# balazs-bamer/cdpr-simulation

Measured on AMD Instinct MI355X. Metric: CDPR sim-steps/sec (whole node), 65 536 parallel 8-cable robots, 1 ms dt, higher is better.
Workload: dtype f32

## Files before the change

cdpr-simulation_amd/csrc/cdpr_engine.hip:

```cpp
#include "cdpr_engine_internal.hpp"

namespace {
thread_local std::string g_create_error;
}

namespace cdpr_host {

int derivative_weights(uint32_t n, uint32_t degree, double* w) {
  if (n < 2 || n > CDPR_MAX_D_BUFFER || degree < 1 || degree > CDPR_MAX_D_DEGREE || degree >= n) return CDPR_ERR_INVALID;
  const int m = (int)degree + 1;
  long double a[5][10];
  for (int i = 0; i < m; ++i)
    for (int j = 0; j < 2 * m; ++j) a[i][j] = 0.0L;
  std::vector<long double> x(n);
  for (uint32_t j = 0; j < n; ++j) x[j] = (long double)j - (long double)(n - 1) / 2.0L;
  for (int i = 0; i < m; ++i) {
    for (int k = 0; k < m; ++k) {
      long double s = 0;
      for (uint32_t j = 0; j < n; ++j) s += powl(x[j], i + k);
      a[i][k] = s;
    }
    a[i][m + i] = 1.0L;
  }
  for (int col = 0; col < m; ++col) {
// ... 497 lines not shown
  HIP_TRY(h, hipMemcpyAsync(c.d_mask, mask.data(), B, hipMemcpyHostToDevice, h->stream));
  HIP_TRY(h, wait_stream(h));
  c.pending = true;
  c.masked = true;
  return CDPR_OK;
}

static int set_command(cdpr_engine* h, int kind, const float* axes, size_t count, bool from_device) {
  if (!h) return CDPR_ERR_INVALID;
  const int rc = stage_command(h, kind, axes, count, from_device);
  if (rc == CDPR_OK) {
    CmdChannel& c = h->cmd[kind];
    c.pending = true;
    c.masked = false;
    c.ext[1] = nullptr;
  }
  return rc;
}

static int bind_command(cdpr_engine* h, int kind, const float* d_axes, size_t count) {
  if (!h) return CDPR_ERR_INVALID;
  if (!d_axes) {
    h->err = "null command buffer";
    return CDPR_ERR_INVALID;
  }
  if (count != (size_t)h->n * h->batch) return CDPR_IGNORED;
  if (h->plan.per_robot) {
    h->err = "cdpr_bind_*_command_device: not available on a per_robot_commands handle (commands are latched robot by robot)";
    return CDPR_ERR_UNSUPPORTED;
  }
  h->cmd[kind].ext[1] = d_axes;
  h->cmd[kind].pending = true;
  return CDPR_OK;
}

int cdpr_set_velocity_command(cdpr_handle_t h, const float* axes, size_t count) { return set_command(h, CDPR_COMMAND_VELOCITY, axes, count, false); }
int cdpr_set_position_command(cdpr_handle_t h, const float* axes, size_t count) { return set_command(h, CDPR_COMMAND_POSITION, axes, count, false); }
int cdpr_set_force_command(cdpr_handle_t h, const float* axes, size_t count) { return set_command(h, CDPR_COMMAND_FORCE, axes, count, false); }

int cdpr_set_velocity_command_device(cdpr_handle_t h, const float* d_axes, size_t count) { return set_command(h, CDPR_COMMAND_VELOCITY, d_axes, count, true); }
int cdpr_set_position_command_device(cdpr_handle_t h, const float* d_axes, size_t count) { return set_command(h, CDPR_COMMAND_POSITION, d_axes, count, true); }
int cdpr_set_force_command_device(cdpr_handle_t h, const float* d_axes, size_t count) { return set_command(h, CDPR_COMMAND_FORCE, d_axes, count, true); }

int cdpr_set_velocity_command_masked(cdpr_handle_t h, const float* axes, size_t count, const uint8_t* robot_mask) {
  return stage_masked(h, CDPR_COMMAND_VELOCITY, axes, count, robot_mask);
}
int cdpr_set_position_command_masked(cdpr_handle_t h, const float* axes, size_t count, const uint8_t* robot_mask) {
  return stage_masked(h, CDPR_COMMAND_POSITION, axes, count, robot_mask);
}
int cdpr_set_force_command_masked(cdpr_handle_t h, const float* axes, size_t count, const uint8_t* robot_mask) {
  return stage_masked(h, CDPR_COMMAND_FORCE, axes, count, robot_mask);
}

int cdpr_bind_velocity_command_device(cdpr_handle_t h, const float* d_axes, size_t count) { return bind_command(h, CDPR_COMMAND_VELOCITY, d_axes, count); }
int cdpr_bind_position_command_device(cdpr_handle_t h, const float* d_axes, size_t count) { return bind_command(h, CDPR_COMMAND_POSITION, d_axes, count); }
int cdpr_bind_force_command_device(cdpr_handle_t h, const float* d_axes, size_t count) { return bind_command(h, CDPR_COMMAND_FORCE, d_axes, count); }

int cdpr_update(cdpr_handle_t h, int nsteps) { return run_steps(h, nsteps, 1); }

int cdpr_update_fused(cdpr_handle_t h, int nsteps, int steps_per_launch) { return run_steps(h, nsteps, steps_per_launch); }

int cdpr_observable_image_bytes(cdpr_handle_t h, size_t* bytes) {
  if (!h || !bytes) return CDPR_ERR_INVALID;
  *bytes = image_bytes(h);
  return CDPR_OK;
}

int cdpr_update_record(cdpr_handle_t h, int nsteps, int steps_per_launch, void* d_record, size_t record_bytes) {
  if (!h) return CDPR_ERR_INVALID;
  if (h->cfg.publish_period != 0.0) {
    h->err = "cdpr_update_record needs publish_period == 0 (every step published)";
    return CDPR_ERR_UNSUPPORTED;
  }
  const size_t image = image_bytes(h);
  if (!d_record || nsteps < 0 || record_bytes < image * (size_t)nsteps) {
    h->err = "cdpr_update_record: record buffer missing or smaller than nsteps observable images";
    return CDPR_ERR_INVALID;
  }
  return run_steps(h, nsteps, steps_per_launch, d_record);
}

int cdpr_update_scheduled(cdpr_handle_t h, int nsteps, int refresh_steps, const float* d_commands, const uint32_t* d_ready, void* d_record,
                          size_t record_bytes) {
  if (!h) return CDPR_ERR_INVALID;
  return scheduled_update(h, CDPR_COMMAND_VELOCITY, nsteps, refresh_steps, d_commands, d_ready, nullptr, d_record, record_bytes);
}

int cdpr_update_scheduled_kind(cdpr_handle_t h, uint32_t kind, int nsteps, int refresh_steps, const float* d_commands, const uint32_t* d_ready,
                               const uint8_t* d_robot_masks, void* d_record, size_t record_bytes) {
  if (!h) return CDPR_ERR_INVALID;
  return scheduled_update(h, kind, nsteps, refresh_steps, d_commands, d_ready, d_robot_masks, d_record, record_bytes);
}

int cdpr_synchronize(cdpr_handle_t h) {
  if (!h) return CDPR_ERR_INVALID;
  if (set_device(h) != CDPR_OK) return CDPR_ERR_DEVICE;
  HIP_TRY(h, wait_stream(h));
  return checked(h, CDPR_OK);
}

static int copy_name(const std::string& text, char* name, size_t len) {
  if (!name || len == 0) return CDPR_ERR_INVALID;
  const size_t k = std::min(text.size(), len - 1);
  memcpy(name, text.data(), k);
  name[k] = 0;
  return CDPR_OK;
}

static LaunchShape shape_of_flags(int steps_per_launch, uint32_t flags) {
  LaunchShape s;
  s.steps = steps_per_launch;
  s.first_world = (flags & CDPR_PLAN_FIRST_WORLD_STEP) != 0u;
  s.scheduled = (flags & CDPR_PLAN_SCHEDULED) != 0u;
  s.rollout = (flags & CDPR_PLAN_ROLLOUT) != 0u;
  s.steady = (flags & CDPR_PLAN_NOT_STEADY) == 0u;
  return s;
}

int cdpr_plan_kernel(const cdpr_config_t* cfg, int steps_per_launch, uint32_t flags, char* name, size_t len) {
  if (!cfg || !name || len == 0 || steps_per_launch < 1) return CDPR_ERR_INVALID;
  const KernelPlan plan = plan_kernels(*cfg);
  if (plan.rc != CDPR_OK) {
    copy_name(plan.error, name, len);
    return plan.rc;
  }
  return copy_name(planned_kernel_name(planned_kernel(plan, shape_of_flags(steps_per_launch, flags))), name, len);
}

int cdpr_debug_plan_entry(const cdpr_config_t* cfg, int steps_per_launch, uint32_t flags) {
  if (!cfg || steps_per_launch < 1) return CDPR_ERR_INVALID;
  const KernelPlan plan = plan_kernels(*cfg);
  if (plan.rc != CDPR_OK) return plan.rc;
  return missing_entry(plan, shape_of_flags(steps_per_launch, flags)).id == KernelId::None ? 1 : 0;
}
const void* cdpr_debug_plan_entry_address(const cdpr_config_t* cfg, int steps_per_launch, uint32_t flags) {
  if (!cfg || steps_per_launch < 1) return nullptr;
  const KernelPlan plan = plan_kernels(*cfg);
  return plan.rc != CDPR_OK ? nullptr : entry_address(planned_kernel(plan, shape_of_flags(steps_per_launch, flags)));
}

int cdpr_kernel_name(cdpr_handle_t h, char* name, size_t len) {
  if (!h) return CDPR_ERR_INVALID;
  return copy_name(planned_kernel_name(h->last_kernel), name, len);
}

uint32_t cdpr_mapping(cdpr_handle_t h) {
  return !h ? CDPR_MAP_AUTO : (h->plan.lane_cable ? CDPR_MAP_LANE_PER_CABLE : h->plan.lane_pair ? CDPR_MAP_LANE_PAIR : CDPR_MAP_LANE_PER_ROBOT);
}

uint64_t cdpr_step_count(cdpr_handle_t h) { return h ? h->step : 0; }

int cdpr_debug_last_variant(cdpr_handle_t h) { return h ? (h->last_kernel.steady ? 1 : 0) : -1; }

#ifdef CDPR_STAMPS
int cdpr_debug_set_stamps(cdpr_handle_t h, unsigned long long* d_stamps) {
  if (!h) return CDPR_ERR_INVALID;
  h->base.stamps = d_stamps;
  return CDPR_OK;
}
#endif

int cdpr_device_malloc(cdpr_handle_t h, size_t bytes, void** out) {
  if (!h || !out) return CDPR_ERR_INVALID;
  if (set_device(h) != CDPR_OK) return CDPR_ERR_DEVICE;
  HIP_TRY(h, hipMalloc(out, bytes));
  return CDPR_OK;
}

int cdpr_device_free(cdpr_handle_t h, void* ptr) {
  if (!h) return CDPR_ERR_INVALID;
  if (set_device(h) != CDPR_OK) return CDPR_ERR_DEVICE;
  HIP_TRY(h, hipFree(ptr));
  return CDPR_OK;
}

int cdpr_device_upload(cdpr_handle_t h, void* dst, const void* src, size_t bytes) {
  if (!h || !dst || !src) return CDPR_ERR_INVALID;
  if (set_device(h) != CDPR_OK) return CDPR_ERR_DEVICE;
  HIP_TRY(h, hipMemcpyAsync(dst, src, bytes, hipMemcpyHostToDevice, h->stream));
  HIP_TRY(h, wait_stream(h));
  return CDPR_OK;
}

int cdpr_device_download(cdpr_handle_t h, void* dst, const void* src, size_t bytes) {
  if (!h || !dst || !src) return CDPR_ERR_INVALID;
  if (set_device(h) != CDPR_OK) return CDPR_ERR_DEVICE;
  HIP_TRY(h, hipMemcpyAsync(dst, src, bytes, hipMemcpyDeviceToHost, h->stream));
  HIP_TRY(h, wait_stream(h));
  return checked(h, CDPR_OK);
}

int cdpr_profile_begin(cdpr_handle_t h) {
  if (!h) return CDPR_ERR_INVALID;
  if (set_device(h) != CDPR_OK) return CDPR_ERR_DEVICE;
  h->launches_mark = h->launches;
  HIP_TRY(h, hipEventRecord(h->ev0, h->stream));
  return CDPR_OK;
}

int cdpr_profile_end(cdpr_handle_t h, float* elapsed_ms, uint64_t* kernel_launches) {
  if (!h) return CDPR_ERR_INVALID;
  if (set_device(h) != CDPR_OK) return CDPR_ERR_DEVICE;
  HIP_TRY(h, hipEventRecord(h->ev1, h->stream));
  HIP_TRY(h, wait_stream(h));
  float ms = 0.f;
  HIP_TRY(h, hipEventElapsedTime(&ms, h->ev0, h->ev1));
  if (elapsed_ms) *elapsed_ms = ms;
  if (kernel_launches) *kernel_launches = h->launches - h->launches_mark;
  return CDPR_OK;
}

}
```

cdpr-simulation_amd/csrc/cdpr_onestep_kernel.hpp:

```cpp
#pragma once
#include "cdpr_step_kernel.hpp"

namespace cdpr {

CDPR_DEV void row_to_lds(const float4* src, float4* dst_row) {
  __builtin_amdgcn_global_load_lds((const __attribute__((address_space(1))) void*)src, (__attribute__((address_space(3))) void*)dst_row, 16, 0, 0);
}


template <int NP, bool PR = false, bool FULL = false>
CDPR_DEV void pid_pairs(const StepArgs& a, int calls, bool is_vel, const v2f (&desired)[NP], const v2f (&actual)[NP], const v2f (&win)[NP][kWin],
                        v2f (&ierr)[NP], v2f (&f)[NP], v2f (&e_new)[NP], float& dbg_p, float& dbg_i, float& dbg_d, bool is_force = false) {
  const PidCoef c = pid_coef<PR>(a, is_vel);
  const bool run = (!PR || calls != 0) && !is_force;
  const bool full = FULL || calls >= c.nbuf;
  const float (&wt)[kWin + 2] = a.wrow;
  v2f error[NP], acc[NP];
#pragma unroll
  for (int k = 0; k < NP; ++k) {
    error[k] = desired[k] - actual[k];
    acc[k] = splat(wt[kWin]) * error[k];
  }
#pragma unroll
  for (int j = 0; j < kWin; ++j) {
// ... 228 lines not shown
      ierr[2 * g] = (v2f){h.x, h.y};
      if (2 * g + 1 < NP) ierr[2 * g + 1] = (v2f){h.z, h.w};
    }
    const bool actual_is_vel = (a.flags & kFlagActualIsVelocity) != 0u;
    v2f actual[NP];
#pragma unroll
    for (int k = 0; k < NP; ++k) actual[k] = actual_is_vel ? qd[k] : q[k];
    const int ring_slot = a.ring_slot;
    pid_pairs<NP>(a, a.pid_calls, actual_is_vel, desired, actual, win, ierr, f, e_new, dbg_p, dbg_i, dbg_d);
    dbg_wrote = true;
    if (live) {
#pragma unroll
      for (int m = 0; m < 5; ++m) {
        if (m == (ring_slot >> 1)) {
#pragma unroll
          for (int k = 0; k < NP; ++k) CDPR_STORE_STATE(a.state, st, P + 5 * k + m, woff, ring_row(win[k], m, e_new[k], ring_slot));
        }
      }
#pragma unroll
      for (int g = 0; g < NH; ++g) {
        const int k1 = (2 * g + 1 < NP) ? 2 * g + 1 : 2 * g;
        CDPR_STORE_STATE(a.state, st, P + 5 * NP + g, woff, make_float4(ierr[2 * g].x, ierr[2 * g].y, ierr[k1].x, ierr[k1].y));
      }
    }
  }

  if (force_mode && !first_world) {
#pragma unroll
    for (int k = 0; k < NP; ++k) f[k] = desired[k];
  }

  if (PERSIST && more) {
    const uint32_t noff = nrr * 16u;
    if (run_pid) {
#pragma unroll
      for (int j = 0; j < kCtrl; ++j)
        row_to_lds(reinterpret_cast<const float4*>(reinterpret_cast<const char*>(a.state + (size_t)(P + j) * st) + noff), &stage[j][0]);
      if (kCmdLds) {
        const float* ncp = a.cmd + (size_t)nrr * N;
#pragma unroll
        for (int g = 0; g < kCmdRows; ++g) row_to_lds(reinterpret_cast<const float4*>(ncp) + g, &stage[kCtrl + g][0]);
      }
    }
  }

  CDPR_STAMP(5);
  v2f applied[NP];
  int td_flag = 0;
  if (TD) {
    v2f df[NP];
#pragma unroll
    for (int k = 0; k < NP; ++k) df[k] = f[k] - splat(a.td_mid);
    float g[6];
    if (FK) {
      jt_times<NP>(jest, df, g);
      normal_solve<NP, false>(jest, 0.f, g);
    } else {
      jt_times<NP>(jac, df, g);
      normal_solve<NP, false>(jac, 0.f, g);
    }
#pragma unroll
    for (int k = 0; k < NP; ++k) {
      v2f t = splat(a.td_mid);
#pragma unroll
      for (int c = 0; c < 6; ++c) t = fma2(g[c], FK ? jest[k][c] : jac[k][c], t);
      const v2f tc = max2(min2(t, splat(a.td_max)), splat(a.td_min));
      td_flag |= (tc.x != t.x) ? 1 : 0;
      if (2 * k + 1 < N) td_flag |= (tc.y != t.y) ? 1 : 0;
      applied[k] = tc;
    }
  } else {
#pragma unroll
    for (int k = 0; k < NP; ++k) applied[k] = f[k];
  }
  setforce_limits<NP>(a, qd, applied);

  if (a.dbg && live) write_pid_topic(a.dbg + (size_t)r * 9, dbg_wrote, dbg_wrote, dbg_p, dbg_i, dbg_d, desired[0].x, applied[0].x);
  if (publish && live) {
    store_slot(a.obs, st, 3, woff, make_float4(s.wz, fk_res, (float)fk_it, pack_flags(td_flag, travel_mask<N>(a, q))));
#pragma unroll
    for (int g = 0; g < G; ++g) {
      const int k0 = 2 * g, k1 = (2 * g + 1 < NP) ? 2 * g + 1 : 2 * g;
      const bool has = (2 * g + 1 < NP);
      store_slot(a.obs, st, 4 + 2 * G + g, woff,
                make_float4(applied[k0].x, applied[k0].y, has ? applied[k1].x : 0.f, has ? applied[k1].y : 0.f));
    }
  }

  CDPR_STAMP(6);
  {
    v2f tens[NP];
#pragma unroll
    for (int k = 0; k < NP; ++k) {
      tens[k] = fma2(-a.damping, qd[k], applied[k]);
      if (a.unilateral) tens[k] = max2(tens[k], splat(0.f));
    }
    if (FK) {
      uint32_t again = 0;
      asm volatile("" : "+v"(again));
      v2f len2[NP], l02[NP];
      ik_pairs<N, false>(lds + again, s.px, s.py, s.pz, s.qx, s.qy, s.qz, s.qw, len2, jac, l02);
    }
    float w[6];
    jt_times<NP>(jac, tens, w);
    w[0] = a.fgx - w[0];
    w[1] = a.fgy - w[1];
    w[2] = a.fgz - w[2];
    w[3] = -w[3];
    w[4] = -w[4];
    w[5] = -w[5];
    integrate(a, s, w);
  }
  if (PERSIST && more) {
    constexpr int kDmaOps = kCtrl + kCmdRows;
    static_assert(kDmaOps < 64, "vmcnt is a 6-bit counter");
    if (run_pid)
      __builtin_amdgcn_s_waitcnt(vmcnt_imm(kDmaOps));
    else
      __builtin_amdgcn_s_waitcnt(vmcnt_imm(0));
    asm volatile("" : "+a"(n0), "+a"(n1), "+a"(n2), "+a"(n3), "+a"(n4));
  }
  if (live) {
    CDPR_STORE_STATE(a.state, st, 0, woff, make_float4(s.px, s.py, s.pz, s.qx));
    CDPR_STORE_STATE(a.state, st, 1, woff, make_float4(s.qy, s.qz, s.qw, s.vx));
    CDPR_STORE_STATE(a.state, st, 2, woff, make_float4(s.vy, s.vz, s.wx, s.wy));
    CDPR_STORE_STATE(a.state, st, 3, woff, make_float4(s.wz, fkx, fky, fkz));
    if (FK) CDPR_STORE_STATE(a.state, st, 4, woff, make_float4(fkqx, fkqy, fkqz, fkqw));
  }
  CDPR_STAMP(7);
  if (!(PERSIST && more)) break;
  blk = nblk;
  r = nr;
  rr = nrr;
  live = r < a.batch;
  off = rr * 16u, woff = r * 16u;
  p0 = make_float4(n0.x, n0.y, n0.z, n0.w), p1 = make_float4(n1.x, n1.y, n1.z, n1.w), p2 = make_float4(n2.x, n2.y, n2.z, n2.w);
  p3 = make_float4(n3.x, n3.y, n3.z, n3.w), p4 = make_float4(n4.x, n4.y, n4.z, n4.w);
  staged = run_pid;
  }
}

#ifndef CDPR_CTL_LOAD_DELAY
#define CDPR_CTL_LOAD_DELAY 8
#endif
#ifndef CDPR_SPLIT_PRIO
#define CDPR_SPLIT_PRIO 1
#endif
#ifndef CDPR_STEADY_SHARED_IK
#define CDPR_STEADY_SHARED_IK 1
#endif
#ifndef CDPR_STEADY_NEWTON_WRITTEN_OUT
#define CDPR_STEADY_NEWTON_WRITTEN_OUT 1
#endif
constexpr int kIkRows = 7;
#ifdef CDPR_STAMPS
#define CDPR_SPLIT_STAMP(i)                                                                                          \
  do {                                                                                                               \
    __builtin_amdgcn_sched_barrier(0);                                                                               \
    if (a.stamps && lane == 0) a.stamps[(size_t)blockIdx.x * 8 + (i)] = __builtin_amdgcn_s_memrealtime();           \
    __builtin_amdgcn_sched_barrier(0);                                                                               \
  } while (0)
#else
#define CDPR_SPLIT_STAMP(i) do { } while (0)
#endif
#if defined(CDPR_STAMPS) && defined(CDPR_STAMPS_ITER)
#define CDPR_CTL_STAMP(i) do { } while (0)
#else
#define CDPR_CTL_STAMP(i) CDPR_SPLIT_STAMP(i)
#endif

template <int N, int XS, int ES, bool RAISED = true, bool STEADY = false>
CDPR_DEV void split_estimator_wave(const StepArgs& a, float* geo, float gval, uint32_t lane, bool live, size_t st, uint32_t off, uint32_t woff,
                                   const float4& p0, const float4& p1, const float4& p3, const v2f* x_force, v2f* x_tension, float* x_est,
                                   v2f* x_ik = nullptr) {
  constexpr int NP = cable_pairs(N);
#if defined(CDPR_STAMPS) && defined(CDPR_STAMPS_CLOCK)
  const unsigned long long clk0 = __builtin_amdgcn_s_memtime();
#endif
#if CDPR_SPLIT_PRIO == 1 || CDPR_SPLIT_PRIO == 4
  if (RAISED) __builtin_amdgcn_s_setprio(3);
#elif CDPR_SPLIT_PRIO == 3 || CDPR_SPLIT_PRIO == 5
  if (RAISED) __builtin_amdgcn_s_setprio(2);
#endif
  const float4 p4 = load_slot(a.state, st, 4, off);
  if (lane < NP * kGeomFloatsPerPair) geo[lane] = gval;
  __builtin_amdgcn_fence(__ATOMIC_RELEASE, "wavefront");
  __builtin_amdgcn_wave_barrier();
  __builtin_amdgcn_fence(__ATOMIC_ACQUIRE, "wavefront");
  float fkx = p3.y, fky = p3.z, fkz = p3.w, fkqx = p4.x, fkqy = p4.y, fkqz = p4.z, fkqw = p4.w;
  v2f len[NP];
  {
    v2f jac[NP][6], l0[NP];
    ik_pairs<N, false>(geo, p0.x, p0.y, p0.z, p0.w, p1.x, p1.y, p1.z, len, jac, l0);
    if (STEADY && CDPR_STEADY_SHARED_IK) {
#pragma unroll
      for (int k = 0; k < NP; ++k) {
        x_ik[(kIkRows * k) * 64 + lane] = len[k];
#pragma unroll
        for (int c = 0; c < 6; ++c) x_ik[(kIkRows * k + 1 + c) * 64 + lane] = jac[k][c];
      }
      __builtin_amdgcn_fence(__ATOMIC_RELEASE, "workgroup");
      __builtin_amdgcn_s_waitcnt(0xC07F);
      __builtin_amdgcn_s_barrier();
    }
  }
  float fk_res = 0.f;
  int fk_it = 0;
  v2f jest[NP][6];
  {
    v2f elen[NP], unused[NP];
    if (STEADY && CDPR_STEADY_NEWTON_WRITTEN_OUT) {
#pragma unroll
      for (int it = 0; it < 4; ++it) {
        ik_pairs<N, false>(geo, fkx, fky, fkz, fkqx, fkqy, fkqz, fkqw, elen, jest, unused);
        v2f res[NP];
#pragma unroll
        for (int k = 0; k < NP; ++k) res[k] = len[k] - elen[k];
        float g[6];
        jt_times<NP>(jest, res, g);
        normal_solve<NP>(jest, a.fk_lambda, g);
        fkx += g[0];
        fky += g[1];
        fkz += g[2];
        quat_apply_rotvec(fkqx, fkqy, fkqz, fkqw, g[3], g[4], g[5]);
#ifdef CDPR_STAMPS_ITER
        if (it < 3) {
          asm volatile("" ::"v"(fkqw));
          __builtin_amdgcn_sched_barrier(0);
          if (a.stamps && lane == 0) a.stamps[(size_t)blockIdx.x * 8 + 4 + it] = __builtin_amdgcn_s_memrealtime();
          __builtin_amdgcn_sched_barrier(0);
        }
#endif
      }
      fk_it = 4;
    } else {
      bool active = true;
      for (int it = 0; it < a.fk_iters; ++it) {
        ik_pairs<N, false>(geo, fkx, fky, fkz, fkqx, fkqy, fkqz, fkqw, elen, jest, unused);
        v2f res[NP];
        v2f rm = splat(0.f);
#pragma unroll
        for (int k = 0; k < NP; ++k) {
          res[k] = len[k] - elen[k];
          rm = max2(rm, abs2(res[k]));
        }
        active = active && !(fmaxf(rm.x, rm.y) < a.fk_tol);
        float g[6];
        jt_times<NP>(jest, res, g);
        normal_solve<NP>(jest, a.fk_lambda, g);
        if (active) {
          fkx += g[0];
          fky += g[1];
          fkz += g[2];
          quat_apply_rotvec(fkqx, fkqy, fkqz, fkqw, g[3], g[4], g[5]);
          ++fk_it;
        }
#ifdef CDPR_STAMPS_ITER
        if (it < 3) {
          asm volatile("" ::"v"(fkqw));
          __builtin_amdgcn_sched_barrier(0);
          if (a.stamps && lane == 0) a.stamps[(size_t)blockIdx.x * 8 + 4 + it] = __builtin_amdgcn_s_memrealtime();
          __builtin_amdgcn_sched_barrier(0);
        }
#endif
      }
    }
    ik_pairs<N, false>(geo, fkx, fky, fkz, fkqx, fkqy, fkqz, fkqw, elen, jest, unused);
    v2f rm = splat(0.f);
#pragma unroll
    for (int k = 0; k < NP; ++k) rm = max2(rm, abs2(len[k] - elen[k]));
    fk_res = fmaxf(rm.x, rm.y);
  }
  if (live) store_slot_aux<CDPR_SPLIT_PLAT_AUX>(a.state, st, 4, woff, make_float4(fkqx, fkqy, fkqz, fkqw));
  CDPR_SPLIT_STAMP(1);
  v2f td_l[6][3];
  float td_invd[6];
  normal_matrix_pk<NP, false>(jest, 0.f, td_l);
  chol_factor_pk(td_l, td_invd);
  __builtin_amdgcn_s_waitcnt(0xC07F);
  __builtin_amdgcn_s_barrier();
  CDPR_SPLIT_STAMP(2);
  __builtin_amdgcn_fence(__ATOMIC_ACQUIRE, "workgroup");
  v2f f[NP], df[NP], t_out[NP];
#pragma unroll
  for (int k = 0; k < NP; ++k) {
    f[k] = x_force[k * XS + lane];
    df[k] = f[k] - splat(a.td_mid);
  }
  int td_flag = 0;
  {
    float g[6];
    jt_times<NP>(jest, df, g);
    chol_apply_pk(td_l, td_invd, g);
#pragma unroll
    for (int k = 0; k < NP; ++k) {
      v2f t = splat(a.td_mid);
#pragma unroll
      for (int c = 0; c < 6; ++c) t = fma2(g[c], jest[k][c], t);
      const v2f tc = max2(min2(t, splat(a.td_max)), splat(a.td_min));
      td_flag |= (tc.x != t.x) ? 1 : 0;
      if (2 * k + 1 < N) td_flag |= (tc.y != t.y) ? 1 : 0;
      t_out[k] = tc;
    }
  }
#pragma unroll
  for (int k = 0; k < NP; ++k) x_tension[k * XS + lane] = t_out[k];
  x_est[0 * ES + lane] = fkx;
  x_est[1 * ES + lane] = fky;
  x_est[2 * ES + lane] = fkz;
  x_est[3 * ES + lane] = fk_res;
  x_est[4 * ES + lane] = (float)fk_it;
  x_est[5 * ES + lane] = (float)td_flag;
  __builtin_amdgcn_fence(__ATOMIC_RELEASE, "workgroup");
  __builtin_amdgcn_s_waitcnt(0xC07F);
  CDPR_SPLIT_STAMP(3);
#if defined(CDPR_STAMPS) && defined(CDPR_STAMPS_CLOCK)
  if (a.stamps && lane == 0) a.stamps[(size_t)blockIdx.x * 8 + 7] = __builtin_amdgcn_s_memtime() - clk0;
#endif
  __builtin_amdgcn_s_barrier();
}

template <int N, bool PR, bool STEADY, bool VEL>
CDPR_DEV void split_controller_wave(const StepArgs& a, float* geo, float gval, uint32_t lane, uint32_t r, uint32_t rr, bool live, size_t st, uint32_t off,
                                    uint32_t woff, const float4& p0, const float4& p1, const float4& p2, const float4& p3, v2f* x_force, const v2f* x_tension,
                                    const float* x_est, const v2f* x_ik = nullptr) {
  static_assert(!(STEADY && PR), "the steady instantiation serves uniform handles");
  constexpr int NP = cable_pairs(N);
  constexpr int P = plat_slots(true);
  constexpr int G = joint_groups(N);
  constexpr int NH = (NP + 1) / 2;
#if CDPR_SPLIT_PRIO == 2 || CDPR_SPLIT_PRIO == 5
  __builtin_amdgcn_s_setprio(3);
#endif
#if CDPR_CTL_LOAD_DELAY > 0
  __builtin_amdgcn_s_sleep(CDPR_CTL_LOAD_DELAY);
#endif
  float4 wraw[NP][5], hraw[NH];
#pragma unroll
  for (int k = 0; k < NP; ++k) {
#pragma unroll
    for (int m = 0; m < 5; ++m) wraw[k][m] = load_slot(a.state, st, P + 5 * k + m, off);
  }
#pragma unroll
  for (int g = 0; g < NH; ++g) hraw[g] = load_slot(a.state, st, P + 5 * NP + g, off);
  v2f desired[NP];
#pragma unroll
  for (int k = 0; k < NP; ++k) desired[k] = splat(0.f);
  const float* cp = a.cmd + (size_t)rr * N;
  if (N % 4 == 0) {
#pragma unroll
    for (int g = 0; g < N / 4; ++g) {
      const float4 v = reinterpret_cast<const float4*>(cp)[g];
      desired[2 * g] = (v2f){v.x, v.y};
      desired[2 * g + 1] = (v2f){v.z, v.w};
    }
  } else {
#pragma unroll
    for (int i = 0; i < N; ++i) {
      if (i & 1)
        desired[i / 2].y = cp[i];
      else
        desired[i / 2].x = cp[i];
    }
  }
  if (lane < NP * kGeomFloatsPerPair) geo[lane] = gval;
  __builtin_amdgcn_fence(__ATOMIC_RELEASE, "wavefront");
  __builtin_amdgcn_wave_barrier();
  __builtin_amdgcn_fence(__ATOMIC_ACQUIRE, "wavefront");

  Platform s;
  unpack_platform(p0, p1, p2, p3.x, s);

  v2f len[NP], q[NP], qd[NP], jac[NP][6];
  {
    v2f l0[NP];
    if (STEADY && CDPR_STEADY_SHARED_IK) {
      __builtin_amdgcn_s_barrier();
      __builtin_amdgcn_fence(__ATOMIC_ACQUIRE, "workgroup");
#pragma unroll
      for (int k = 0; k < NP; ++k) {
        len[k] = x_ik[(kIkRows * k) * 64 + lane];
#pragma unroll
        for (int c = 0; c < 6; ++c) jac[k][c] = x_ik[(kIkRows * k + 1 + c) * 64 + lane];
        l0[k] = *reinterpret_cast<const v2f*>(geo + k * kGeomFloatsPerPair + 12);
      }
    } else {
      ik_pairs<N, true>(geo, s.px, s.py, s.pz, s.qx, s.qy, s.qz, s.qw, len, jac, l0);
    }
#pragma unroll
    for (int k = 0; k < NP; ++k) {
      q[k] = l0[k] - len[k];
      qd[k] = -fma2(s.wz, jac[k][5], fma2(s.wy, jac[k][4], fma2(s.wx, jac[k][3],
                    fma2(s.vz, jac[k][2], fma2(s.vy, jac[k][1], splat(s.vx) * jac[k][0])))));
    }
  }
  const bool publish = STEADY || (a.publish_mask & 1ull) != 0ull;
  if (publish && live) {
    store_slot(a.obs, st, 0, woff, make_float4(s.px, s.py, s.pz, s.qx));
    store_slot(a.obs, st, 1, woff, make_float4(s.qy, s.qz, s.qw, s.vx));
    store_slot(a.obs, st, 2, woff, make_float4(s.vy, s.vz, s.wx, s.wy));
#pragma unroll
    for (int g = 0; g < G; ++g) {
      const int k0 = 2 * g, k1 = (2 * g + 1 < NP) ? 2 * g + 1 : 2 * g;
      const bool has = (2 * g + 1 < NP);
      store_slot(a.obs, st, 4 + g, woff, make_float4(q[k0].x, q[k0].y, has ? q[k1].x : 0.f, has ? q[k1].y : 0.f));
      store_slot(a.obs, st, 4 + G + g, woff, make_float4(qd[k0].x, qd[k0].y, has ? qd[k1].x : 0.f, has ? qd[k1].y : 0.f));
    }
  }

  v2f f[NP], e_new[NP], ierr[NP];
#pragma unroll
  for (int k = 0; k < NP; ++k) {
    f[k] = splat(0.f);
    e_new[k] = splat(0.f);
    ierr[k] = (k & 1) ? (v2f){hraw[k / 2].z, hraw[k / 2].w} : (v2f){hraw[k / 2].x, hraw[k / 2].y};
  }
  float dbg_p = 0.f, dbg_i = 0.f, dbg_d = 0.f;
  bool dbg_wrote = false;
  const bool first_world = !STEADY && (a.flags & kFlagFirstWorldStep) != 0u;
  uint32_t meta = 0u;
  if (PR) meta = a.meta[rr];
  const int calls = PR ? (int)(meta >> kMetaCallShift) : a.pid_calls;
  if (PR && live && !first_world) a.meta[r] = (uint8_t)((meta & kMetaModeMask) | ((uint32_t)min(calls + 1, (int)kMetaCallMax) << kMetaCallShift));
  const bool force_mode = !STEADY && !PR && (a.flags & kFlagForceMode) != 0u;
  if (force_mode && !first_world) {
#pragma unroll
    for (int k = 0; k < NP; ++k) f[k] = desired[k];
  } else if (STEADY || (!first_world && (PR || calls != 0))) {
    v2f win[NP][kWin];
#pragma unroll
    for (int k = 0; k < NP; ++k) {
#pragma unroll
      for (int m = 0; m < 5; ++m) {
        win[k][2 * m] = (v2f){wraw[k][m].x, wraw[k][m].y};
        win[k][2 * m + 1] = (v2f){wraw[k][m].z, wraw[k][m].w};
      }
    }
    const bool actual_is_vel = STEADY ? VEL : PR ? ((meta & kMetaModeMask) == kMetaVelocity) : ((a.flags & kFlagActualIsVelocity) != 0u);
    v2f actual[NP];
#pragma unroll
    for (int k = 0; k < NP; ++k) actual[k] = actual_is_vel ? qd[k] : q[k];
    const int ring_slot = a.ring_slot;
    const bool is_force = PR && (meta & kMetaModeMask) == kMetaForce;
#if CDPR_SPLIT_PRIO == 3 || CDPR_SPLIT_PRIO == 4
    __builtin_amdgcn_s_setprio(3);
#endif
    pid_pairs<NP, PR, STEADY>(a, calls, actual_is_vel, desired, actual, win, ierr, f, e_new, dbg_p, dbg_i, dbg_d, is_force);
    dbg_wrote = (!PR || calls != 0) && !is_force;
    if (live) {
#pragma unroll
      for (int m = 0; m < 5; ++m) {
        if (m == (ring_slot >> 1)) {
          if (!STEADY) {
#pragma unroll
            for (int k = 0; k < NP; ++k) CDPR_STORE_STATE(a.state, st, P + 5 * k + m, woff, ring_row(win[k], m, e_new[k], ring_slot));
          } else if (ring_slot & 1) {
#pragma unroll
            for (int k = 0; k < NP; ++k) CDPR_STORE_STATE(a.state, st, P + 5 * k + m, woff, make_float4(win[k][2 * m].x, win[k][2 * m].y, e_new[k].x, e_new[k].y));
          } else {
#pragma unroll
            for (int k = 0; k < NP; ++k) CDPR_STORE_STATE(a.state, st, P + 5 * k + m, woff, make_float4(e_new[k].x, e_new[k].y, win[k][2 * m + 1].x, win[k][2 * m + 1].y));
          }
        }
      }
#pragma unroll
      for (int g = 0; g < NH; ++g) {
        const int k1 = (2 * g + 1 < NP) ? 2 * g + 1 : 2 * g;
        CDPR_STORE_STATE(a.state, st, P + 5 * NP + g, woff, make_float4(ierr[2 * g].x, ierr[2 * g].y, ierr[k1].x, ierr[k1].y));
      }
    }
  }
#pragma unroll
  for (int k = 0; k < NP; ++k) x_force[k * 64 + lane] = f[k];
  __builtin_amdgcn_fence(__ATOMIC_RELEASE, "workgroup");
  __builtin_amdgcn_s_waitcnt(0xC07F);
  CDPR_CTL_STAMP(4);
#if CDPR_SPLIT_PRIO >= 3
  __builtin_amdgcn_s_setprio(0);
#endif
  __builtin_amdgcn_s_barrier();
  __builtin_amdgcn_s_barrier();
  CDPR_CTL_STAMP(5);
  __builtin_amdgcn_fence(__ATOMIC_ACQUIRE, "workgroup");
  v2f applied[NP];
#pragma unroll
  for (int k = 0; k < NP; ++k) applied[k] = x_tension[k * 64 + lane];
  const float fkx = x_est[0 * 64 + lane], fky = x_est[1 * 64 + lane], fkz = x_est[2 * 64 + lane], fk_res = x_est[3 * 64 + lane],
              fk_it = x_est[4 * 64 + lane], td_flag = x_est[5 * 64 + lane];
  setforce_limits<NP>(a, qd, applied);
  if (!STEADY && a.dbg && live) write_pid_topic(a.dbg + (size_t)r * 9, dbg_wrote, dbg_wrote, dbg_p, dbg_i, dbg_d, desired[0].x, applied[0].x);
  if (publish && live) {
    store_slot(a.obs, st, 3, woff, make_float4(s.wz, fk_res, fk_it, (!STEADY && a.travel_on) ? pack_flags((int)td_flag, travel_mask<N>(a, q)) : td_flag));
#pragma unroll
    for (int g = 0; g < G; ++g) {
      const int k0 = 2 * g, k1 = (2 * g + 1 < NP) ? 2 * g + 1 : 2 * g;
      const bool has = (2 * g + 1 < NP);
      store_slot(a.obs, st, 4 + 2 * G + g, woff,
                 make_float4(applied[k0].x, applied[k0].y, has ? applied[k1].x : 0.f, has ? applied[k1].y : 0.f));
    }
  }
  {
    v2f tens[NP];
#pragma unroll
    for (int k = 0; k < NP; ++k) {
      tens[k] = fma2(-a.damping, qd[k], applied[k]);
      if (a.unilateral) tens[k] = max2(tens[k], splat(0.f));
    }
    float w[6];
    jt_times<NP>(jac, tens, w);
    w[0] = a.fgx - w[0];
    w[1] = a.fgy - w[1];
    w[2] = a.fgz - w[2];
    w[3] = -w[3];
    w[4] = -w[4];
    w[5] = -w[5];
    integrate(a, s, w);
  }
  if (live) {
    store_slot_aux<CDPR_SPLIT_PLAT_AUX>(a.state, st, 0, woff, make_float4(s.px, s.py, s.pz, s.qx));
    store_slot_aux<CDPR_SPLIT_PLAT_AUX>(a.state, st, 1, woff, make_float4(s.qy, s.qz, s.qw, s.vx));
    store_slot_aux<CDPR_SPLIT_PLAT_AUX>(a.state, st, 2, woff, make_float4(s.vy, s.vz, s.wx, s.wy));
    store_slot_aux<CDPR_SPLIT_PLAT_AUX>(a.state, st, 3, woff, make_float4(s.wz, fkx, fky, fkz));
  }
  CDPR_CTL_STAMP(6);
}

template <int N, bool PR, bool STEADY, bool VEL>
CDPR_DEV void split_kernel_body(const StepArgs& a) {
  constexpr int NP = cable_pairs(N);
  __shared__ __attribute__((aligned(16))) float lds[2][NP * kGeomFloatsPerPair];
  __shared__ v2f x_force[NP][64];
  __shared__ v2f x_tension[NP][64];
  __shared__ float x_est[6][64];
  v2f* x_ik = nullptr;
  if constexpr (STEADY && CDPR_STEADY_SHARED_IK) {
    __shared__ v2f ik_rows_at_state[kIkRows * NP][64];
    x_ik = &ik_rows_at_state[0][0];
  }

  const uint32_t swap = __builtin_popcount(blockIdx.x & a.split_swap) & 1u;
  const uint32_t wave = (threadIdx.x >> 6) ^ swap, lane = threadIdx.x & 63u;
  const uint32_t r = blockIdx.x * 64u + lane;
  const uint32_t rr = (r < a.batch) ? r : (a.batch - 1u);
  const bool live = r < a.batch;
  const size_t st = a.stride;
  const uint32_t off = rr * 16u, woff = r * 16u;
  float* const geo = lds[wave];

  if (wave == 0) CDPR_SPLIT_STAMP(0);
#ifdef CDPR_STAMPS
  if (a.stamps && lane == 0)
    reinterpret_cast<uint32_t*>(&a.stamps[(size_t)blockIdx.x * 8 + 7])[threadIdx.x >> 6] =
        (__builtin_amdgcn_s_getreg((16 - 1) << 11 | 4) & 0xffffu) | ((__builtin_amdgcn_s_getreg((4 - 1) << 11 | 20) & 0xfu) << 16);
#endif
  const float gval = (lane < NP * kGeomFloatsPerPair) ? a.geom[lane] : 0.f;
  const float4 p0 = load_slot(a.state, st, 0, off), p1 = load_slot(a.state, st, 1, off), p2 = load_slot(a.state, st, 2, off),
               p3 = load_slot(a.state, st, 3, off);
  if (wave == 0) {
    split_estimator_wave<N, 64, 64, true, STEADY>(a, geo, gval, lane, live, st, off, woff, p0, p1, p3, &x_force[0][0], &x_tension[0][0], &x_est[0][0], x_ik);
    return;
  }
  split_controller_wave<N, PR, STEADY, VEL>(a, geo, gval, lane, r, rr, live, st, off, woff, p0, p1, p2, p3, &x_force[0][0], &x_tension[0][0], &x_est[0][0], x_ik);
}
template <int N, bool PR = false>
__global__ __launch_bounds__(128, 2) void cdpr_split_kernel(const StepArgs a) { split_kernel_body<N, PR, false, false>(a); }
template <int N, bool VEL>
__global__ __launch_bounds__(128, 2) void cdpr_split_steady_kernel(const StepArgs a) { split_kernel_body<N, false, true, VEL>(a); }

}
```

Before: 6.739 billion.

## Share rotation matrix via LDS, pin FMA chains, and store PID ring halves

```diff
diff --git a/cdpr-simulation_amd/csrc/cdpr_engine.hip b/cdpr-simulation_amd/csrc/cdpr_engine.hip
--- a/cdpr-simulation_amd/csrc/cdpr_engine.hip
+++ b/cdpr-simulation_amd/csrc/cdpr_engine.hip
@@ -673,6 +673,14 @@
 
 int cdpr_debug_last_variant(cdpr_handle_t h) { return h ? (h->last_kernel.steady ? 1 : 0) : -1; }
 
+int cdpr_debug_slot_rows(cdpr_handle_t h, const void** state, const void** obs, uint32_t* n_state, uint32_t* n_obs, uint32_t* stride) {
+  if (!h || !state || !obs || !n_state || !n_obs || !stride) return CDPR_ERR_INVALID;
+  if (h->plan.fp64) return CDPR_ERR_UNSUPPORTED;
+  *state = h->d_state.p, *obs = h->d_obs.p;
+  *n_state = (uint32_t)h->n_state, *n_obs = (uint32_t)h->n_obs, *stride = h->stride;
+  return CDPR_OK;
+}
+
 #ifdef CDPR_STAMPS
 int cdpr_debug_set_stamps(cdpr_handle_t h, unsigned long long* d_stamps) {
   if (!h) return CDPR_ERR_INVALID;
diff --git a/cdpr-simulation_amd/csrc/cdpr_onestep_kernel.hpp b/cdpr-simulation_amd/csrc/cdpr_onestep_kernel.hpp
--- a/cdpr-simulation_amd/csrc/cdpr_onestep_kernel.hpp
+++ b/cdpr-simulation_amd/csrc/cdpr_onestep_kernel.hpp
@@ -404,7 +404,160 @@
 #ifndef CDPR_STEADY_NEWTON_WRITTEN_OUT
 #define CDPR_STEADY_NEWTON_WRITTEN_OUT 1
 #endif
+#ifndef CDPR_STEADY_ROT_PLAIN
+#define CDPR_STEADY_ROT_PLAIN 1
+#endif
+#ifndef CDPR_STEADY_SHARED_ROT
+#define CDPR_STEADY_SHARED_ROT 1
+#endif
+#ifndef CDPR_STEADY_STEP_PLAIN
+#define CDPR_STEADY_STEP_PLAIN 1
+#endif
+#ifndef CDPR_STEADY_PAIR_STORES
+#define CDPR_STEADY_PAIR_STORES 1
+#endif
+template <bool PLAIN>
+CDPR_LEAF float pin_if(float v) {
+  if constexpr (PLAIN) asm("" : "+v"(v));
+  return v;
+}
+template <bool PLAIN>
+CDPR_LEAF float fma_p(float a, float b, float c) { return pin_if<PLAIN>(fmaf(a, b, c)); }
+template <bool PLAIN>
+CDPR_LEAF float mul_p(float a, float b) { return pin_if<PLAIN>(a * b); }
+
+template <bool PLAIN>
+CDPR_DEV Rot quat_to_rot_p(float x, float y, float z, float w) {
+  if constexpr (!PLAIN) return quat_to_rot(x, y, z, w);
+  constexpr auto P = pin_if<PLAIN>;
+  const float x2 = P(x + x), y2 = P(y + y), z2 = P(z + z);
+  const float xx = P(x * x2), yy = P(y * y2), zz = P(z * z2);
+  const float xy = P(x * y2), xz = P(x * z2), yz = P(y * z2);
+  const float wx = P(w * x2), wy = P(w * y2), wz = P(w * z2);
+  Rot r;
+  r.r00 = P(1.f - P(yy + zz));
+  r.r01 = P(xy - wz);
+  r.r02 = P(xz + wy);
+  r.r10 = P(xy + wz);
+  r.r11 = P(1.f - P(xx + zz));
+  r.r12 = P(yz - wx);
+  r.r20 = P(xz - wy);
+  r.r21 = P(yz + wx);
+  r.r22 = P(1.f - P(xx + yy));
+  return r;
+}
+
+template <int N>
+CDPR_DEV void ik_pairs_rot(const float* lds, float px, float py, float pz, const Rot& r, v2f (&len)[cable_pairs(N)], v2f (&jac)[cable_pairs(N)][6]) {
+  constexpr int NP = cable_pairs(N);
+#pragma unroll
+  for (int k = 0; k < NP; ++k) {
+    const float4 g0 = *reinterpret_cast<const float4*>(lds + k * kGeomFloatsPerPair);
+    const float4 g1 = *reinterpret_cast<const float4*>(lds + k * kGeomFloatsPerPair + 4);
+    const float4 g2 = *reinterpret_cast<const float4*>(lds + k * kGeomFloatsPerPair + 8);
+    const v2f ax = {g0.x, g0.y}, ay = {g0.z, g0.w}, az = {g1.x, g1.y};
+    const v2f bx = {g1.z, g1.w}, by = {g2.x, g2.y}, bz = {g2.z, g2.w};
+    const v2f rbx = fma2(r.r02, bz, fma2(r.r01, by, splat(r.r00) * bx));
+    const v2f rby = fma2(r.r12, bz, fma2(r.r11, by, splat(r.r10) * bx));
+    const v2f rbz = fma2(r.r22, bz, fma2(r.r21, by, splat(r.r20) * bx));
+    const v2f lx = (rbx - ax) + splat(px), ly = (rby - ay) + splat(py), lz = (rbz - az) + splat(pz);
+    const v2f l2 = fma2(lz, lz, fma2(ly, ly, lx * lx));
+    const v2f inv = rsq2(l2);
+    len[k] = l2 * inv;
+    const v2f ux = lx * inv, uy = ly * inv, uz = lz * inv;
+    jac[k][0] = ux;
+    jac[k][1] = uy;
+    jac[k][2] = uz;
+    jac[k][3] = fma2(rby, uz, -(rbz * uy));
+    jac[k][4] = fma2(rbz, ux, -(rbx * uz));
+    jac[k][5] = fma2(rbx, uy, -(rby * ux));
+    if ((N & 1) && k == NP - 1) {
+      const float4 g3 = *reinterpret_cast<const float4*>(lds + k * kGeomFloatsPerPair + 12);
+      const v2f mask = {g3.z, g3.w};
+      len[k] *= mask;
+#pragma unroll
+      for (int c = 0; c < 6; ++c) jac[k][c] *= mask;
+    }
+  }
+}
+
+template <bool PLAIN>
+CDPR_DEV void quat_apply_rotvec_p(float& qx, float& qy, float& qz, float& qw, float tx, float ty, float tz) {
+  constexpr auto F = fma_p<PLAIN>;
+  constexpr auto M = mul_p<PLAIN>;
+  const float a2 = fmaf(tz, tz, fmaf(ty, ty, tx * tx));
+  const float inv_a = __frsqrt_rn(fmaxf(a2, 1e-30f));
+  float s, c;
+  __sincosf(0.5f * (a2 * inv_a), &s, &c);
+  const bool tiny = a2 < 1e-8f;
+  const float k = tiny ? fmaf(a2, -1.f / 48.f, 0.5f) : s * inv_a;
+  const float cw = tiny ? fmaf(a2, -0.125f, 1.f) : c;
+  const float dx = M(k, tx), dy = M(k, ty), dz = M(k, tz);
+  const float nw = F(-dz, qz, F(-dy, qy, F(-dx, qx, M(cw, qw))));
+  const float nx = F(-dz, qy, F(dy, qz, F(qw, dx, M(cw, qx))));
+  const float ny = F(-dx, qz, F(dz, qx, F(qw, dy, M(cw, qy))));
+  const float nz = F(-dy, qx, F(dx, qy, F(qw, dz, M(cw, qz))));
+  const float inv = __frsqrt_rn(F(nw, nw, F(nz, nz, F(ny, ny, M(nx, nx)))));
+  qx = M(nx, inv);
+  qy = M(ny, inv);
+  qz = M(nz, inv);
+  qw = M(nw, inv);
+}
+
+template <bool PLAIN>
+CDPR_DEV void integrate_velocity_rot(const StepArgs& a, Platform& s, const float (&w)[6], const Rot& r) {
+  constexpr auto F = fma_p<PLAIN>;
+  constexpr auto M = mul_p<PLAIN>;
+  s.vx = F(a.dt_inv_mass, w[0], s.vx);
+  s.vy = F(a.dt_inv_mass, w[1], s.vy);
+  s.vz = F(a.dt_inv_mass, w[2], s.vz);
+  float tbx = F(r.r20, w[5], F(r.r10, w[4], M(r.r00, w[3])));
+  float tby = F(r.r21, w[5], F(r.r11, w[4], M(r.r01, w[3])));
+  float tbz = F(r.r22, w[5], F(r.r12, w[4], M(r.r02, w[3])));
+  const float obx = F(r.r20, s.wz, F(r.r10, s.wy, M(r.r00, s.wx)));
+  const float oby = F(r.r21, s.wz, F(r.r11, s.wy, M(r.r01, s.wx)));
+  const float obz = F(r.r22, s.wz, F(r.r12, s.wy, M(r.r02, s.wx)));
+  const float iox = F(a.ib[4], obz, F(a.ib[3], oby, M(a.ib[0], obx)));
+  const float ioy = F(a.ib[5], obz, F(a.ib[1], oby, M(a.ib[3], obx)));
+  const float ioz = F(a.ib[2], obz, F(a.ib[5], oby, M(a.ib[4], obx)));
+  tbx = pin_if<PLAIN>(tbx - F(oby, ioz, -M(obz, ioy)));
+  tby = pin_if<PLAIN>(tby - F(obz, iox, -M(obx, ioz)));
+  tbz = pin_if<PLAIN>(tbz - F(obx, ioy, -M(oby, iox)));
+  const float abx = F(a.ibinv[4], tbz, F(a.ibinv[3], tby, M(a.ibinv[0], tbx)));
+  const float aby = F(a.ibinv[5], tbz, F(a.ibinv[1], tby, M(a.ibinv[3], tbx)));
+  const float abz = F(a.ibinv[2], tbz, F(a.ibinv[5], tby, M(a.ibinv[4], tbx)));
+  s.wx = F(a.dt, F(r.r02, abz, F(r.r01, aby, M(r.r00, abx))), s.wx);
+  s.wy = F(a.dt, F(r.r12, abz, F(r.r11, aby, M(r.r10, abx))), s.wy);
+  s.wz = F(a.dt, F(r.r22, abz, F(r.r21, aby, M(r.r20, abx))), s.wz);
+}
+
+template <bool PLAIN>
+CDPR_DEV void integrate_pose_p(const StepArgs& a, Platform& s) {
+  if constexpr (!PLAIN) return integrate_pose(a, s);
+  constexpr auto F = fma_p<PLAIN>;
+  constexpr auto M = mul_p<PLAIN>;
+  s.px = F(a.dt, s.vx, s.px);
+  s.py = F(a.dt, s.vy, s.py);
+  s.pz = F(a.dt, s.vz, s.pz);
+  const float h = a.half_dt;
+  const float nx = F(h, F(-s.wz, s.qy, F(s.wy, s.qz, M(s.qw, s.wx))), s.qx);
+  const float ny = F(h, F(-s.wx, s.qz, F(s.wz, s.qx, M(s.qw, s.wy))), s.qy);
+  const float nz = F(h, F(-s.wy, s.qx, F(s.wx, s.qy, M(s.qw, s.wz))), s.qz);
+  const float nw = F(-h, F(s.wz, s.qz, F(s.wy, s.qy, M(s.wx, s.qx))), s.qw);
+  const float inv = __frsqrt_rn(F(nw, nw, F(nz, nz, F(ny, ny, M(nx, nx)))));
+  s.qx = M(nx, inv);
+  s.qy = M(ny, inv);
+  s.qz = M(nz, inv);
+  s.qw = M(nw, inv);
+}
+
+__device__ void raw_buffer_store_v2f(v2f data, __amdgpu_buffer_rsrc_t rsrc, int voffset, int soffset, int aux) __asm("llvm.amdgcn.raw.ptr.buffer.store.v2f32");
+CDPR_DEV void store_slot_half(float4* base, size_t stride, int slot, uint32_t off, int half, v2f v) {
+  const auto rsrc = __builtin_amdgcn_make_buffer_rsrc(base + (size_t)slot * stride, 0, (int)(stride * sizeof(float4)), 0x00020000);
+  raw_buffer_store_v2f(v, rsrc, (int)off, half, CDPR_STORE_AUX);
+}
 constexpr int kIkRows = 7;
+constexpr int kRotRows = 9;
 #ifdef CDPR_STAMPS
 #define CDPR_SPLIT_STAMP(i)                                                                                          \
   do {                                                                                                               \
@@ -424,8 +577,10 @@
 template <int N, int XS, int ES, bool RAISED = true, bool STEADY = false>
 CDPR_DEV void split_estimator_wave(const StepArgs& a, float* geo, float gval, uint32_t lane, bool live, size_t st, uint32_t off, uint32_t woff,
                                    const float4& p0, const float4& p1, const float4& p3, const v2f* x_force, v2f* x_tension, float* x_est,
-                                   v2f* x_ik = nullptr) {
+                                   v2f* x_ik = nullptr, float* x_rot = nullptr) {
   constexpr int NP = cable_pairs(N);
+  constexpr bool kPlain = STEADY && CDPR_STEADY_ROT_PLAIN;
+  constexpr bool kRotOut = STEADY && CDPR_STEADY_SHARED_IK && CDPR_STEADY_SHARED_ROT;
 #if defined(CDPR_STAMPS) && defined(CDPR_STAMPS_CLOCK)
   const unsigned long long clk0 = __builtin_amdgcn_s_memtime();
 #endif
@@ -443,7 +598,17 @@
   v2f len[NP];
   {
     v2f jac[NP][6], l0[NP];
-    ik_pairs<N, false>(geo, p0.x, p0.y, p0.z, p0.w, p1.x, p1.y, p1.z, len, jac, l0);
+    if constexpr (kPlain || kRotOut) {
+      const Rot rot = quat_to_rot_p<kPlain>(p0.w, p1.x, p1.y, p1.z);
+      ik_pairs_rot<N>(geo, p0.x, p0.y, p0.z, rot, len, jac);
+      if (kRotOut) {
+        const float rm[kRotRows] = {rot.r00, rot.r01, rot.r02, rot.r10, rot.r11, rot.r12, rot.r20, rot.r21, rot.r22};
+#pragma unroll
+        for (int c = 0; c < kRotRows; ++c) x_rot[c * 64 + lane] = rm[c];
+      }
+    } else {
+      ik_pairs<N, false>(geo, p0.x, p0.y, p0.z, p0.w, p1.x, p1.y, p1.z, len, jac, l0);
+    }
     if (STEADY && CDPR_STEADY_SHARED_IK) {
 #pragma unroll
       for (int k = 0; k < NP; ++k) {
@@ -464,7 +629,10 @@
     if (STEADY && CDPR_STEADY_NEWTON_WRITTEN_OUT) {
 #pragma unroll
       for (int it = 0; it < 4; ++it) {
-        ik_pairs<N, false>(geo, fkx, fky, fkz, fkqx, fkqy, fkqz, fkqw, elen, jest, unused);
+        if constexpr (kPlain)
+          ik_pairs_rot<N>(geo, fkx, fky, fkz, quat_to_rot_p<true>(fkqx, fkqy, fkqz, fkqw), elen, jest);
+        else
+          ik_pairs<N, false>(geo, fkx, fky, fkz, fkqx, fkqy, fkqz, fkqw, elen, jest, unused);
         v2f res[NP];
 #pragma unroll
         for (int k = 0; k < NP; ++k) res[k] = len[k] - elen[k];
@@ -474,7 +642,10 @@
         fkx += g[0];
         fky += g[1];
         fkz += g[2];
-        quat_apply_rotvec(fkqx, fkqy, fkqz, fkqw, g[3], g[4], g[5]);
+        if constexpr (kPlain)
+          quat_apply_rotvec_p<true>(fkqx, fkqy, fkqz, fkqw, g[3], g[4], g[5]);
+        else
+          quat_apply_rotvec(fkqx, fkqy, fkqz, fkqw, g[3], g[4], g[5]);
 #ifdef CDPR_STAMPS_ITER
         if (it < 3) {
           asm volatile("" ::"v"(fkqw));
@@ -517,7 +688,10 @@
 #endif
       }
     }
-    ik_pairs<N, false>(geo, fkx, fky, fkz, fkqx, fkqy, fkqz, fkqw, elen, jest, unused);
+    if constexpr (kPlain)
+      ik_pairs_rot<N>(geo, fkx, fky, fkz, quat_to_rot_p<true>(fkqx, fkqy, fkqz, fkqw), elen, jest);
+    else
+      ik_pairs<N, false>(geo, fkx, fky, fkz, fkqx, fkqy, fkqz, fkqw, elen, jest, unused);
     v2f rm = splat(0.f);
 #pragma unroll
     for (int k = 0; k < NP; ++k) rm = max2(rm, abs2(len[k] - elen[k]));
@@ -575,7 +749,7 @@
 template <int N, bool PR, bool STEADY, bool VEL>
 CDPR_DEV void split_controller_wave(const StepArgs& a, float* geo, float gval, uint32_t lane, uint32_t r, uint32_t rr, bool live, size_t st, uint32_t off,
                                     uint32_t woff, const float4& p0, const float4& p1, const float4& p2, const float4& p3, v2f* x_force, const v2f* x_tension,
-                                    const float* x_est, const v2f* x_ik = nullptr) {
+                                    const float* x_est, const v2f* x_ik = nullptr, const float* x_rot = nullptr) {
   static_assert(!(STEADY && PR), "the steady instantiation serves uniform handles");
   constexpr int NP = cable_pairs(N);
   constexpr int P = plat_slots(true);
@@ -699,10 +873,16 @@
 #endif
     pid_pairs<NP, PR, STEADY>(a, calls, actual_is_vel, desired, actual, win, ierr, f, e_new, dbg_p, dbg_i, dbg_d, is_force);
     dbg_wrote = (!PR || calls != 0) && !is_force;
+    if (STEADY && CDPR_STEADY_PAIR_STORES) {
+      if (live) {
+#pragma unroll
+        for (int k = 0; k < NP; ++k) store_slot_half(a.state, st, P + 5 * k + (ring_slot >> 1), woff, (ring_slot & 1) * 8, e_new[k]);
+      }
+    }
     if (live) {
 #pragma unroll
       for (int m = 0; m < 5; ++m) {
-        if (m == (ring_slot >> 1)) {
+        if (m == (ring_slot >> 1) && !(STEADY && CDPR_STEADY_PAIR_STORES)) {
           if (!STEADY) {
 #pragma unroll
             for (int k = 0; k < NP; ++k) CDPR_STORE_STATE(a.state, st, P + 5 * k + m, woff, ring_row(win[k], m, e_new[k], ring_slot));
@@ -766,7 +946,17 @@
     w[3] = -w[3];
     w[4] = -w[4];
     w[5] = -w[5];
-    integrate(a, s, w);
+    if constexpr (STEADY && CDPR_STEADY_SHARED_IK && CDPR_STEADY_SHARED_ROT) {
+      const Rot rot = {x_rot[0 * 64 + lane], x_rot[1 * 64 + lane], x_rot[2 * 64 + lane], x_rot[3 * 64 + lane], x_rot[4 * 64 + lane],
+                       x_rot[5 * 64 + lane], x_rot[6 * 64 + lane], x_rot[7 * 64 + lane], x_rot[8 * 64 + lane]};
+      integrate_velocity_rot<CDPR_STEADY_STEP_PLAIN != 0>(a, s, w, rot);
+      integrate_pose_p<CDPR_STEADY_STEP_PLAIN != 0>(a, s);
+    } else if constexpr (STEADY && CDPR_STEADY_STEP_PLAIN) {
+      integrate_velocity_rot<true>(a, s, w, quat_to_rot_p<true>(s.qx, s.qy, s.qz, s.qw));
+      integrate_pose_p<true>(a, s);
+    } else {
+      integrate(a, s, w);
+    }
   }
   if (live) {
     store_slot_aux<CDPR_SPLIT_PLAT_AUX>(a.state, st, 0, woff, make_float4(s.px, s.py, s.pz, s.qx));
@@ -789,6 +979,11 @@
     __shared__ v2f ik_rows_at_state[kIkRows * NP][64];
     x_ik = &ik_rows_at_state[0][0];
   }
+  float* x_rot = nullptr;
+  if constexpr (STEADY && CDPR_STEADY_SHARED_IK && CDPR_STEADY_SHARED_ROT) {
+    __shared__ float rot_at_state[kRotRows][64];
+    x_rot = &rot_at_state[0][0];
+  }
 
   const uint32_t swap = __builtin_popcount(blockIdx.x & a.split_swap) & 1u;
   const uint32_t wave = (threadIdx.x >> 6) ^ swap, lane = threadIdx.x & 63u;
@@ -809,10 +1004,10 @@
   const float4 p0 = load_slot(a.state, st, 0, off), p1 = load_slot(a.state, st, 1, off), p2 = load_slot(a.state, st, 2, off),
                p3 = load_slot(a.state, st, 3, off);
   if (wave == 0) {
-    split_estimator_wave<N, 64, 64, true, STEADY>(a, geo, gval, lane, live, st, off, woff, p0, p1, p3, &x_force[0][0], &x_tension[0][0], &x_est[0][0], x_ik);
+    split_estimator_wave<N, 64, 64, true, STEADY>(a, geo, gval, lane, live, st, off, woff, p0, p1, p3, &x_force[0][0], &x_tension[0][0], &x_est[0][0], x_ik, x_rot);
     return;
   }
-  split_controller_wave<N, PR, STEADY, VEL>(a, geo, gval, lane, r, rr, live, st, off, woff, p0, p1, p2, p3, &x_force[0][0], &x_tension[0][0], &x_est[0][0], x_ik);
+  split_controller_wave<N, PR, STEADY, VEL>(a, geo, gval, lane, r, rr, live, st, off, woff, p0, p1, p2, p3, &x_force[0][0], &x_tension[0][0], &x_est[0][0], x_ik, x_rot);
 }
 template <int N, bool PR = false>
 __global__ __launch_bounds__(128, 2) void cdpr_split_kernel(const StepArgs a) { split_kernel_body<N, PR, false, false>(a); }
```

New measurement: 6.733 billion. No clear change (-0.1%).
